# Luolin0826/band

Hardware: AMD Instinct MI355X
Metric: multi-DNN inferences/sec + p99 job latency, 4-model int8 mix @1/2/4/8 GPU (higher is better)
Workload: dtype int8

## Files before the change

band_amd/_abi.py:

```python
import ctypes
import os

_HERE = os.path.dirname(os.path.abspath(__file__))
LIB_PATH = os.path.join(_HERE, "libband_hip%s.so" % (
    "_" + os.environ["BAND_HIP_LIB_VARIANT"] if os.environ.get("BAND_HIP_LIB_VARIANT") else ""))

c_int, c_int32, c_void_p, c_size_t = ctypes.c_int, ctypes.c_int32, ctypes.c_void_p, ctypes.c_size_t


class ConvParams(ctypes.Structure):
    _fields_ = [(n, c_int) for n in (
        "batch", "in_h", "in_w", "in_c", "out_h", "out_w", "out_c", "k_h", "k_w",
        "stride_h", "stride_w", "dil_h", "dil_w", "pad_h", "pad_w", "k_pad", "n_pad", "in_xor")] + [
        (n, c_int32) for n in ("in_zp", "w_zp", "out_zp", "act_min", "act_max")] + [
        (n, c_void_p) for n in ("input", "output", "weights", "bias_eff", "mult", "shift", "residual")] + [
        (n, c_int32) for n in ("add_y_off", "add_r_off", "add_o_off", "add_left_shift", "add_y_mult",
                               "add_y_shift", "add_r_mult", "add_r_shift", "add_o_mult", "add_o_shift",
                               "add_act_min", "add_act_max")] + [("out_table", c_void_p), ("requant_fast", c_int32),
                                                                  ("kernel_hint", c_int32),
                                                                  ("out_img_stride", ctypes.c_int64)]


class ConvGroup(ctypes.Structure):
    _fields_ = [("n", c_int), ("blocks", c_int), ("is1x1", c_int), ("table", c_void_p)]
# ... 36 lines not shown
        "has_expand", "tile_h", "tile_w")] + [
        ("exp_w", c_void_p), ("exp_k_pad", c_int), ("exp_bias_eff", c_void_p), ("exp_mult", c_void_p),
        ("exp_shift", c_void_p)] + [(n, c_int32) for n in ("x_zp", "e_zp", "e_act_min", "e_act_max")] + [
        ("dw_w", c_void_p), ("dw_bias", c_void_p), ("dw_mult", c_void_p), ("dw_shift", c_void_p)] + [
        (n, c_int32) for n in ("d_zp", "d_act_min", "d_act_max")] + [
        ("proj_w", c_void_p), ("proj_k_pad", c_int), ("proj_bias_eff", c_void_p), ("proj_mult", c_void_p),
        ("proj_shift", c_void_p)] + [(n, c_int32) for n in ("p_zp", "p_act_min", "p_act_max")] + [
        ("has_residual", c_int)] + [(n, c_int32) for n in (
            "add_p_off", "add_x_off", "add_o_off", "add_left_shift", "add_p_mult", "add_p_shift", "add_x_mult",
            "add_x_shift", "add_o_mult", "add_o_shift", "add_act_min", "add_act_max")] + [
        ("input", c_void_p), ("output", c_void_p), ("debug_stamps", c_void_p), ("requant_fast", c_int32)]


class MeanParams(ctypes.Structure):
    _fields_ = [(n, ctypes.c_long) for n in ("outer", "reduce", "inner")] + [("type", c_int)] + [
        (n, c_int32) for n in ("multiplier", "shift", "bias")] + [("input", c_void_p), ("output", c_void_p)]


class DetectionParams(ctypes.Structure):
    _fields_ = [(n, c_int) for n in ("batch", "num_boxes", "num_classes", "num_classes_with_background",
                                     "max_detections")] + [
        (n, ctypes.c_float) for n in ("score_threshold", "iou_threshold", "scale_y", "scale_x", "scale_h",
                                      "scale_w")] + [
        ("box_type", c_int), ("score_type", c_int), ("box_scale", ctypes.c_float), ("score_scale", ctypes.c_float),
        ("box_zp", c_int32), ("score_zp", c_int32)] + [
        (n, c_void_p) for n in ("box_encodings", "class_scores", "anchors", "out_boxes", "out_classes",
                                "out_scores", "out_num", "scratch")]


class ChainParams(ctypes.Structure):
    _fields_ = [("dw", DwConvParams), ("pw1", ConvParams), ("pw2", ConvParams), ("has_pw2", c_int),
                ("px_blocks", c_int), ("waves", c_int), ("persist", c_int), ("tile", c_int),
                ("tile_blob", c_void_p), ("debug_stamps", c_void_p), ("deep", c_int), ("c_split", c_int),
                ("stage", c_int)]


CONCAT_MAX_INPUTS = 16


class ConcatParams(ctypes.Structure):
    _fields_ = [("n_inputs", c_int), ("outer", ctypes.c_long),
                ("row", ctypes.c_long * CONCAT_MAX_INPUTS), ("input", c_void_p * CONCAT_MAX_INPUTS),
                ("table", c_void_p * CONCAT_MAX_INPUTS), ("output", c_void_p)]


class PadParams(ctypes.Structure):
    _fields_ = [("elem_bytes", c_int), ("in_shape", c_int * 4), ("pad_before", c_int * 4),
                ("pad_after", c_int * 4), ("value", ctypes.c_uint32), ("input", c_void_p), ("output", c_void_p),
                ("mode", c_int32)]


class ResizeNearestParams(ctypes.Structure):
    _fields_ = [(n, c_int) for n in ("batch", "in_h", "in_w", "out_h", "out_w", "row_bytes")] + [
        (n, c_void_p) for n in ("y_index", "x_index", "input", "output")]


class ResizeBilinearParams(ctypes.Structure):
    _fields_ = [(n, c_int) for n in ("batch", "in_h", "in_w", "channels", "out_h", "out_w")] + [
        (n, c_void_p) for n in ("y_tab", "x_tab", "input", "output")]


ARG_I8, ARG_U8, ARG_F32 = 0, 1, 2


class ArgMinMaxParams(ctypes.Structure):
    _fields_ = [(n, ctypes.c_long) for n in ("outer", "axis_len", "inner")] + [
        (n, c_int) for n in ("in_type", "is_min", "out_bytes")] + [("input", c_void_p), ("output", c_void_p)]
# ... 120 lines not shown
    "bh_argminmax_kernel": (ctypes.c_char_p, [ctypes.POINTER(ArgMinMaxParams)]),
    "bh_resize_bilinear_argminmax_i8": (c_int, [ctypes.POINTER(ResizeArgMinMaxParams), c_void_p]),
    "bh_resize_bilinear_argminmax_i8_ok": (c_int, [ctypes.POINTER(ResizeArgMinMaxParams)]),
    "bh_reindex": (c_int, [ctypes.POINTER(ReindexParams), c_void_p]),
    "bh_reindex_as": (c_int, [ctypes.POINTER(ReindexParams), c_int, c_void_p]),
    "bh_reindex_kernel": (ctypes.c_char_p, [ctypes.POINTER(ReindexParams)]),
    "bh_reindex_canonical": (c_int, [ctypes.POINTER(ReindexParams), ctypes.POINTER(ReindexParams)]),
    "bh_softmax_i8": (c_int, [ctypes.POINTER(SoftmaxParams), c_void_p]),
    "bh_zero_insert": (c_int, [ctypes.POINTER(ZeroInsertParams), c_void_p]),
    "bh_conv2d_f32": (c_int, [ctypes.POINTER(ConvF32Params), c_void_p]),
    "bh_conv2d_f32_split": (c_int, [ctypes.POINTER(ConvF32Params)]),
    "bh_fc_f32": (c_int, [ctypes.POINTER(FcF32Params), c_void_p]),
    "bh_eltwise_f32": (c_int, [ctypes.POINTER(EltwiseF32Params), c_void_p]),
    "bh_pool_f32": (c_int, [ctypes.POINTER(PoolF32Params), c_void_p]),
    "bh_unary_f32": (c_int, [c_int, c_void_p, c_void_p, ctypes.c_long, ctypes.c_float, ctypes.c_float, c_void_p]),
    "bh_softmax_f32": (c_int, [c_void_p, c_void_p, ctypes.c_long, c_int, ctypes.c_float, c_void_p]),
    "bh_dwconv2d_i8": (c_int, [ctypes.POINTER(DwConvParams), c_void_p]),
    "bh_fc_i8": (c_int, [ctypes.POINTER(FcParams), c_void_p]),
    "bh_eltwise_i8": (c_int, [ctypes.POINTER(EltwiseParams), c_void_p]),
    "bh_pool_i8": (c_int, [ctypes.POINTER(PoolParams), c_void_p]),
    "bh_irb_i8": (c_int, [ctypes.POINTER(IrbParams), c_void_p]),
    "bh_irb_lds_bytes": (c_size_t, [ctypes.POINTER(IrbParams)]),
    "bh_chain_i8": (c_int, [ctypes.POINTER(ChainParams), c_void_p]),
    "bh_mean": (c_int, [ctypes.POINTER(MeanParams), c_void_p]),
    "bh_detection_scratch_bytes": (c_size_t, [c_int, c_int]),
    "bh_detection_postprocess": (c_int, [ctypes.POINTER(DetectionParams), c_void_p]),
    "bh_chain_lds_bytes": (c_size_t, [ctypes.POINTER(ChainParams)]),
    "bh_chain_tile_lds_bytes": (c_size_t, [ctypes.POINTER(ChainParams)]),
    "bh_chain_tile_launch": (c_int, [ctypes.POINTER(ChainParams), c_void_p]),
    "bh_chain_tile_blob_bytes": (c_size_t, [ctypes.POINTER(ChainParams)]),
    "bh_chain_tile_pack": (c_int, [ctypes.POINTER(ChainParams), c_void_p, c_void_p]),
    "bh_chain_stage_lds_bytes": (c_size_t, [ctypes.POINTER(ChainParams)]),
    "bh_chain_stage_launch": (c_int, [ctypes.POINTER(ChainParams), c_void_p]),
    "bh_last_error": (ctypes.c_char_p, []),
}

BACKEND_SYMBOLS = {}

_lib = None
_configured = set()


class BandHipError(RuntimeError):
    pass


def load():
    global _lib
    if _lib is None:
        if not os.path.exists(LIB_PATH):
            raise BandHipError(
                "libband_hip.so not built (%s); run __graft_entry__.build() / make -C band_amd/csrc" % LIB_PATH)
        _lib = ctypes.CDLL(LIB_PATH)
    for name, (res, args) in list(KERNEL_SYMBOLS.items()) + list(BACKEND_SYMBOLS.items()):
        if name in _configured:
            continue
        fn = getattr(_lib, name)
        fn.restype = res
        fn.argtypes = args
        _configured.add(name)
    return _lib


def check(rc, what=""):
    if rc != 0:
        msg = load().bh_last_error()
# ... 3 lines not shown
```

band_amd/csrc/backend/hip/chain_form.h:

```cpp
#pragma once

#include "band_hip_kernels.h"

namespace band {
namespace hip {

struct ChainForm {
  int launches;
  int px_blocks, waves, persist, tile, deep, c_split, stage;
};
constexpr bool operator==(const ChainForm& a, const ChainForm& b) {
  return a.launches == b.launches && a.px_blocks == b.px_blocks && a.waves == b.waves && a.persist == b.persist &&
         a.tile == b.tile && a.deep == b.deep && a.c_split == b.c_split && a.stage == b.stage;
}
constexpr ChainForm kUnfused{};
constexpr ChainForm kPlainChain{3, 4, 4, 0, 0, 0, 0, 0};

constexpr ChainForm kChainForms[] = {
    {3, 1, 4, 0, 0, 0, 0, 1}, {3, 1, 8, 0, 0, 0, 0, 1}, {3, 2, 4, 0, 0, 0, 0, 1}, {3, 2, 8, 0, 0, 0, 0, 1},
    {3, 1, 8, 0, 0, 0, 2, 1}, {3, 2, 8, 0, 0, 0, 2, 1}, {3, 1, 8, 0, 0, 0, 4, 1}, {3, 1, 8, 0, 0, 0, 8, 1},
    {3, 1, 8, 0, 0, 0, 0, 2}, {3, 2, 8, 0, 0, 0, 0, 2}, {3, 1, 4, 0, 0, 0, 0, 2}, {3, 1, 8, 0, 0, 0, 2, 2},
    {3, 2, 8, 0, 0, 0, 2, 2}, {3, 1, 8, 0, 0, 0, 3, 2}, {3, 1, 8, 0, 0, 0, 4, 2}, {3, 1, 8, 0, 0, 0, 8, 2},
    {3, 4, 4, 0, 0, 0, 0, 0}, {3, 2, 4, 0, 0, 0, 0, 0}, {3, 1, 4, 0, 0, 0, 0, 0}, {3, 1, 8, 0, 0, 0, 0, 0},
    {3, 1, 16, 0, 0, 0, 0, 0},
    {3, 4, 4, 1, 0, 0, 0, 0}, {3, 4, 4, 0, 1, 0, 0, 0}, {3, 4, 4, 0, 3, 0, 0, 0}, {3, 4, 4, 0, 4, 0, 0, 0},
    {3, 2, 4, 0, 0, 1, 0, 0}, {3, 1, 4, 0, 0, 1, 0, 0}, {3, 1, 8, 0, 0, 1, 0, 0},
    {3, 1, 4, 0, 0, 0, 2, 0}, {3, 1, 8, 0, 0, 0, 2, 0}, {3, 2, 4, 0, 0, 0, 2, 0}, {3, 1, 16, 0, 0, 0, 2, 0},
    {3, 1, 4, 0, 0, 0, 3, 0}, {3, 1, 8, 0, 0, 0, 3, 0}, {3, 1, 4, 0, 0, 0, 4, 0}};

constexpr bool HasLaunches(const ChainForm& f, int launches) {
  return launches == 3 || (launches == 2 && !f.stage && f.c_split <= 1);
}
constexpr bool FilteredOut(const ChainForm& f, bool no_tile, bool no_deep, bool no_split, bool no_stage) {
  return f.stage ? no_stage : (f.tile && no_tile) || (f.deep && no_deep) || (f.c_split && no_split);
}

constexpr int Encode(const ChainForm& f) {
  if (f.launches == 0) return 0;
  if (f.stage) return 100000 + 1000 * (f.stage - 1) + 100 * f.c_split + 10 * f.px_blocks + (f.waves == 8 ? 1 : 0);
  return f.px_blocks + (f.launches == 2 ? 10 : 0) + (f.waves == 16 ? 100 : 0) + (f.waves == 8 ? 300 : 0) +
         (f.persist ? 200 : 0) + (f.tile == 1 ? 400 : 0) + (f.tile == 3 ? 600 : 0) + (f.tile == 4 ? 700 : 0) +
         (f.deep ? 1000 : 0) + (f.c_split > 1 ? 2000 * (f.c_split - 1) : 0);
}
inline bool Decode(int code, ChainForm* out) {
  *out = kUnfused;
  if (code == 0) return true;
  for (ChainForm f : kChainForms)
    for (f.launches = 3; f.launches >= 2; --f.launches)
      if (HasLaunches(f, f.launches) && Encode(f) == code) {
        *out = f;
        return true;
      }
  return false;
}

inline void Apply(const ChainForm& f, bh_chain_params* q) {
  q->px_blocks = f.px_blocks;
  q->waves = f.waves;
  q->persist = f.persist;
  q->tile = f.tile;
  q->deep = f.deep;
  q->c_split = f.c_split;
  q->stage = f.stage;
}
inline bool Fits(ChainForm f, bh_chain_params q) {
  Apply(f, &q);
  return bh_chain_lds_bytes(&q) > 0;
}

enum class ForcedChain { kNone, kPlain, kTile, kDeep, kStage };
inline ChainForm ForcedForm(ForcedChain kind, const bh_chain_params& q) {
  ChainForm plain = kPlainChain, want = kPlainChain;
  plain.launches = want.launches = q.has_pw2 ? 3 : 2;
  if (kind == ForcedChain::kTile) want.tile = 1;
  if (kind == ForcedChain::kDeep) want.px_blocks = want.deep = 1;
  if (kind == ForcedChain::kStage && q.has_pw2) {
    want = ChainForm{3, 1, 8, 0, 0, 0, 2, 1};
    ChainForm loader = want;
    loader.stage = 2;
    if (Fits(want, q) && Fits(loader, q)) want = loader;
  }
  return Fits(want, q) ? want : plain;
}

}
}
```

band_amd/csrc/backend/hip/fusion.cc:

```cpp
#include "backend/hip/chain_form.h"
#include "backend/hip/env.h"
#include "backend/hip/executor_internal.h"
#include <mutex>
#include <optional>
#include <unordered_map>

namespace band {
namespace hip {

using namespace ex;

namespace {
bool LaunchIo(const Launch& l, std::vector<const void*>* rd, std::vector<const void*>* wr) {
  switch (l.kind) {
    case Launch::kConv:
      *rd = {l.conv.input, l.conv.residual};
      *wr = {l.conv.output};
      return true;
    case Launch::kDwConv:
      *rd = {l.dw.input};
      *wr = {l.dw.output};
      return true;
    case Launch::kChain:
      *rd = {l.chain.dw.input, l.chain.pw1.residual};
// ... 444 lines not shown
      out.push_back(L[i]);
      continue;
    }
    std::shared_ptr<DeviceBlob> blob3, blob2;
    auto instantiate = [&](const ChainForm& f, bh_chain_params* q) {
      if (f.launches == 3 ? !ok3 : !ok2) return false;
      *q = f.launches == 3 ? c3 : c2;
      Apply(f, q);
      if (bh_chain_lds_bytes(q) == 0) return false;
      return !(f.tile || f.stage) || PackChainTile(q, f.launches == 3 ? &blob3 : &blob2);
    };
    char key[256];
    std::snprintf(key, sizeof(key), "ch%d:%d:%d:%dx%dx%d:s%dd%d:%d:%d:%d:%d:f%d%d%d%d", kChainTuneVersion, ordinal_,
                  tune_batch_ > 0 ? tune_batch_ : D.dw.batch, D.dw.in_h, D.dw.in_w, D.dw.in_c, D.dw.stride_h, D.dw.dil_h,
                  P1.conv.out_c, P1.conv.residual ? 1 : 0, ok3 ? c3.pw2.out_c : 0, ok3 && c3.pw1.output ? 1 : 0,
                  no_tile_chain_, no_deep_chain_, no_split_chain_, no_stage_chain_);
    const bool forced = forced_chain_ != ForcedChain::kNone;
    const std::optional<int> cached = autotune_ && !forced ? TuneLookup(key) : std::nullopt;
    ChainForm form = kUnfused;
    if (forced) {
      form = ForcedForm(forced_chain_, ok3 ? c3 : c2);
    } else if (cached) {
      Decode(*cached, &form);
    } else {
      std::vector<const Launch*> base = {&D, &P1};
      if (ok3) base.push_back(P2);
      double u = -1.0, u_p2 = 0.0;
      if (autotune_) {
        u = TimeLaunches(base, 10);
        if (ok3) u_p2 = TimeLaunches({P2}, 10);
      }
      const bool measured = u > 0 && u_p2 >= 0;
      Fastest best(u);
      for (ChainForm f : kChainForms) {
        if (!measured || FilteredOut(f, no_tile_chain_, no_deep_chain_, no_split_chain_, no_stage_chain_)) continue;
        for (f.launches = 3; f.launches >= 2; --f.launches) {
          Launch F;
          F.kind = Launch::kChain;
          if (!HasLaunches(f, f.launches) || !instantiate(f, &F.chain)) continue;
          const double us = TimeLaunches({&F}, 10);
          const double total = us + (f.launches == 2 && ok3 ? u_p2 : 0.0);
          if (best.Offer(us > 0 ? total : us)) form = f;
        }
      }
      if (measured) TuneStore(key, Encode(form));
      else form = ForcedForm(ForcedChain::kPlain, ok3 ? c3 : c2);
    }
    Launch F;
    F.kind = Launch::kChain;
    F.op_index = D.op_index;
    if (form.launches == 0 || !instantiate(form, &F.chain)) {
      out.push_back(L[i]);
      continue;
    }
    if (F.chain.tile_blob) sg->consts.push_back(form.launches == 3 ? blob3 : blob2);
    const bool three = form.launches == 3;
    F.out_tensor = three ? P2->out_tensor : P1.out_tensor;
    F.kernel = F.chain.stage ? "chain_stage_kernel" : (F.chain.tile ? "chain_tile_kernel" : "chain_kernel");
    const bh_dwconv_params& dw = F.chain.dw;
    const bh_conv_params& a = F.chain.pw1;
    const double px = static_cast<double>(dw.batch) * dw.out_h * dw.out_w;
    F.alg_bytes = static_cast<double>(dw.batch) * dw.in_h * dw.in_w * dw.in_c + 9.0 * dw.out_c + 28.0 * dw.out_c +
                  (a.residual ? px * a.out_c : 0.0) + (a.output ? px * a.out_c : 0.0) +
                  static_cast<double>(a.out_c) * a.in_c + 12.0 * a.out_c;
    F.alg_ops = D.alg_ops + P1.alg_ops;
    if (three) {
      const bh_conv_params& b = F.chain.pw2;
      F.alg_bytes += px * b.out_c + static_cast<double>(b.out_c) * b.in_c + 12.0 * b.out_c;
      F.alg_ops += P2->alg_ops;
      if (!a.output) sg->fused_tensors.insert(P1.out_tensor);
    }
    out.push_back(F);
    sg->fused_tensors.insert(D.out_tensor);
    i += three ? 2 : 1;
  }
  sg->launches.swap(out);
}

namespace {
void** OutSlot(Launch& l) {
  switch (l.kind) {
    case Launch::kChain: return l.chain.has_pw2 ? &l.chain.pw2.output : &l.chain.pw1.output;
    case Launch::kConv: return &l.conv.output;
    case Launch::kDwConv: return &l.dw.output;
    case Launch::kFc: return &l.fc.output;
    case Launch::kEltwise: return &l.elt.out;
    case Launch::kPool: return &l.pool.output;
    case Launch::kIrb: return &l.irb.output;
    case Launch::kLutU8: return &l.dst;
    default: return nullptr;
  }
// ... 144 lines not shown
```

band_amd/csrc/backend/hip/model_executor.cc:

```cpp
#include "backend/hip/model_executor.h"

#include <sys/prctl.h>
#include <time.h>

#include <chrono>
#include <limits>
#include <mutex>
#include <unordered_map>

#include "backend/hip/affinity.h"
#include "backend/hip/completion.h"
#include "backend/hip/env.h"
#include "backend/hip/executor_internal.h"

namespace band {
namespace hip {

using namespace ex;

namespace ex {
thread_local bool t_variant_ctor = false;
}


// ... 249 lines not shown
  const TflModel& d = model.desc();
  meta_.reserve(d.tensors.size());
  for (const TflTensor& t : d.tensors) {
    auto m = std::make_unique<TensorMeta>();
    m->type = t.type;
    m->dims = t.shape;
    m->name = t.name;
    m->bytes = GetDataTypeBytes(t.type) * t.num_elements();
    m->SetQuant(t.scale, t.zero_point, t.quantized_dimension);
    meta_.push_back(std::move(m));
  }
  consumers_.assign(d.tensors.size(), {});
  producer_.assign(d.tensors.size(), -1);
  for (int i = 0; i < static_cast<int>(d.ops.size()); ++i) {
    for (int t : d.ops[i].inputs)
      if (t >= 0) consumers_[t].push_back(i);
    for (int t : d.ops[i].outputs)
      if (t >= 0) producer_[t] = i;
  }
  const char* f = env::Fusion();
  if (f[0] == '0') allow_fusion_ = false;
  if (std::strcmp(f, "noirb") == 0) allow_irb_ = false;
  if (std::strcmp(f, "noadd") == 0) allow_add_ = false;
  if (std::strcmp(f, "nochain") == 0) allow_chain_ = false;
  if (std::strcmp(f, "nogroup") == 0) allow_group_ = false;
  if (std::strcmp(f, "noargmax") == 0) allow_argmax_ = false;
  if (std::strcmp(f, "forcechain") == 0) forced_chain_ = ForcedChain::kPlain;
  if (std::strcmp(f, "forcetile") == 0) forced_chain_ = ForcedChain::kTile;
  if (std::strcmp(f, "notile") == 0) no_tile_chain_ = true;
  if (std::strcmp(f, "nodeep") == 0) no_deep_chain_ = true;
  if (std::strcmp(f, "nosplit") == 0) no_split_chain_ = true;
  if (std::strcmp(f, "forcedeep") == 0) forced_chain_ = ForcedChain::kDeep;
  if (std::strcmp(f, "forcestage") == 0) forced_chain_ = ForcedChain::kStage;
  if (std::strcmp(f, "nostage") == 0) no_stage_chain_ = true;
  if (!env::Autotune()) autotune_ = false;
  return absl::OkStatus();
}

absl::StatusOr<ModelSpec> HipModelExecutor::InvestigateModelSpec(interface::IModel* model) {
  auto* hm = dynamic_cast<HipModel*>(model);
  if (!hm || !hm->IsInitialized()) return absl::InternalError("Failed to investigate model: not a loaded HIP model");
  const TflModel& d = hm->desc();
  const int num_ops = static_cast<int>(d.ops.size());
  std::vector<DataType> tensor_types;
  std::vector<std::set<int>> op_in, op_out;
  for (const TflOperator& op : d.ops) {
    std::set<int> all, ins, outs;
    for (int t : op.inputs) {
      if (t < 0) continue;
      all.insert(t);
      if (!d.tensors[t].is_const()) ins.insert(t);
    }
    for (int t : op.outputs) {
      if (t < 0) continue;
      all.insert(t);
      if (!d.tensors[t].is_const()) outs.insert(t);
    }
    for (int t : all) tensor_types.push_back(d.tensors[t].type);
    op_in.push_back(ins);
    op_out.push_back(outs);
  }
  std::map<DeviceFlag, std::set<int>> unsupported;
  std::set<DeviceFlag> unavailable;
  const bool gpu = DeviceRegistry::Get().GpuAvailable();
  for (size_t f = 0; f < EnumLength<DeviceFlag>(); ++f) {
    const DeviceFlag flag = static_cast<DeviceFlag>(f);
// ... 617 lines not shown
```

band_amd/csrc/kernels/fused_chain.hip:

```cpp
#include <algorithm>

#include "chain_dw.hpp"
#include "common.hpp"

namespace bh {

__device__ __forceinline__ uint32_t pack4(const int32_t v[4]) {
  const uint32_t lo = __builtin_amdgcn_perm((uint32_t)v[1], (uint32_t)v[0], 0x0c0c0400u);
  const uint32_t hi = __builtin_amdgcn_perm((uint32_t)v[3], (uint32_t)v[2], 0x04000c0cu);
  return lo | hi;
}

__device__ __forceinline__ v4i gemm_tile(const bh_conv_params& c, const unsigned char* xrow, int t, int KS, int r16,
                                         int g) {
  const int8_t* wrow = c.weights + (long)(t * 16 + r16) * c.k_pad + g * 16;
  const int nb = t * 16 + 4 * g;
  const int nl = nb < c.out_c ? nb : 0;
  v4i acc = *(const v4i*)(c.bias_eff + nl);
  int k = 0;
  for (; k + 8 <= KS; k += 8) {
    v4i w[8], x[8];
#pragma unroll
    for (int u = 0; u < 8; ++u) {
      w[u] = *(const v4i*)(wrow + (k + u) * 64);
// ... 771 lines not shown
  return c.k_h == 1 && c.k_w == 1 && c.stride_h == 1 && c.stride_w == 1 && c.pad_h == 0 && c.pad_w == 0 &&
         c.in_c == in_c && c.k_pad == (in_c + 63) / 64 * 64 && c.n_pad >= (c.out_c + 15) / 16 * 16 &&
         c.in_xor == 0 && c.w_zp == 0 && !c.out_table && c.out_c > 0 && c.out_c % 4 == 0 && c.weights &&
         c.bias_eff && c.mult && c.shift;
}

}

extern "C" size_t bh_chain_lds_bytes(const bh_chain_params* pp) {
  if (!pp) return 0;
  const bh_chain_params& p = *pp;
  const bh_dwconv_params& d = p.dw;
  if (!p.tile && !p.stage) {
    if (p.px_blocks != 1 && p.px_blocks != 2 && p.px_blocks != 4) return 0;
    if (p.waves != 0 && p.waves != 4 && !((p.waves == 8 || p.waves == 16) && p.px_blocks == 1)) return 0;
  }
  if (d.k_h != 3 || d.k_w != 3 || d.depth_multiplier != 1 || d.in_c != d.out_c || d.out_c % 16 || !d.taps ||
      d.in_xor != 0 || d.w_zp != 0 || d.out_table || !d.input || !d.weights || !d.mult || !d.shift ||
      d.batch <= 0 || d.out_h <= 0 || d.out_w <= 0 || d.stride_h <= 0 || d.stride_w <= 0)
    return 0;
  if (!bh::conv1x1_ok(p.pw1, d.out_c)) return 0;
  const long P = (long)d.batch * d.out_h * d.out_w;
  if (p.pw1.batch * p.pw1.out_h * p.pw1.out_w != P) return 0;
  if (p.has_pw2) {
    if (!bh::conv1x1_ok(p.pw2, p.pw1.out_c) || p.pw2.residual || !p.pw2.output ||
        p.pw2.k_pad > 64 * bh::kXsMax)
      return 0;
    if ((long)p.pw2.batch * p.pw2.out_h * p.pw2.out_w != P) return 0;
  } else if (!p.pw1.output) {
    return 0;
  }
  const long widest = std::max<long>(std::max(d.out_c, p.pw1.out_c), p.has_pw2 ? p.pw2.out_c : 0);
  if (P * widest >= INT32_MAX || (long)d.batch * d.in_h * d.in_w * d.in_c >= INT32_MAX) return 0;
  if (p.stage) return bh_chain_stage_lds_bytes(pp);
  if (p.c_split < 0 || p.c_split > 4) return 0;
  if (p.c_split > 1 && (p.tile || p.persist || p.deep || p.px_blocks > 2 || !p.has_pw2 ||
                        (p.pw2.out_c + 15) / 16 < p.c_split))
    return 0;
  if (p.tile) return bh_chain_tile_lds_bytes(pp);
  if (p.deep && (p.persist || !((p.px_blocks == 1 && (p.waves == 0 || p.waves == 4 || p.waves == 8)) ||
                                (p.px_blocks == 2 && (p.waves == 0 || p.waves == 4)))))
    return 0;
  if (p.persist) {
    if (p.px_blocks != 4 || (p.waves != 0 && p.waves != 4)) return 0;
    const size_t bytes = bh::persist_lds(p).bytes;
    return bytes <= 160 * 1024 ? bytes : 0;
  }
  bh::ChainLds L = bh::chain_lds(p);
  return L.bytes <= 160 * 1024 ? L.bytes : 0;
}

extern "C" int bh_chain_i8(const bh_chain_params* pp, bh_stream_t stream) {
  const size_t lds = bh_chain_lds_bytes(pp);
  if (lds == 0) {
    bh_set_last_error("bh_chain_i8: invalid or unsupported parameters");
    return BH_EINVAL;
  }
  const bh_chain_params& p = *pp;
  if (p.stage) return bh_chain_stage_launch(pp, stream);
  if (p.tile) return bh_chain_tile_launch(pp, stream);
  const int P = p.dw.batch * p.dw.out_h * p.dw.out_w;
  const bh::ChainLds L = bh::chain_lds(p);
  const bool fast = p.dw.requant_fast && p.pw1.requant_fast && (!p.has_pw2 || p.pw2.requant_fast);
  hipStream_t s = (hipStream_t)stream;
  const bool k2 = !p.has_pw2 || p.pw2.k_pad <= 128;
#define BH_CHAIN_CASE(RB)                                                          \
  if (k2) {                                                                        \
    if (fast) bh::launch_chain<RB, true, 2>(p, P, L, lds, s);                     \
    else bh::launch_chain<RB, false, 2>(p, P, L, lds, s);                         \
  } else {                                                                         \
    if (fast) bh::launch_chain<RB, true, bh::kXsMax>(p, P, L, lds, s);            \
    else bh::launch_chain<RB, false, bh::kXsMax>(p, P, L, lds, s);                \
  }
  if (p.persist) {
    if (k2) {
      if (fast) bh::launch_persist<true, 2>(p, P, lds, s);
      else bh::launch_persist<false, 2>(p, P, lds, s);
    } else {
      if (fast) bh::launch_persist<true, bh::kXsMax>(p, P, lds, s);
      else bh::launch_persist<false, bh::kXsMax>(p, P, lds, s);
    }
    return bh_check_launch("chain_persist_kernel");
  }
  if (p.deep) {
#define BH_DEEP(RB, NW)                                                                      \
  if (k2) {                                                                                  \
    if (fast) bh::launch_chain<RB, true, 2, NW, false, 6>(p, P, L, lds, s);                  \
    else bh::launch_chain<RB, false, 2, NW, false, 6>(p, P, L, lds, s);                      \
  } else {                                                                                   \
    if (fast) bh::launch_chain<RB, true, bh::kXsMax, NW, false, 6>(p, P, L, lds, s);         \
    else bh::launch_chain<RB, false, bh::kXsMax, NW, false, 6>(p, P, L, lds, s);             \
// ... 46 lines not shown
```

include/band_hip_kernels.h:

```cpp
#ifndef BAND_HIP_KERNELS_H_
#define BAND_HIP_KERNELS_H_

#include <stddef.h>
#include <stdint.h>

#ifdef __cplusplus
extern "C" {
#endif

#define BH_EINVAL (-1)

typedef void* bh_stream_t;
typedef void* bh_graph_exec_t;
typedef void* bh_event_t;

int bh_device_count(int* count);
int bh_set_device(int ordinal);
int bh_get_device(int* ordinal);
int bh_device_arch(int ordinal, char* buf, size_t cap);
int bh_device_pci_bus_id(int ordinal, char* buf, int cap);
int bh_stream_create(bh_stream_t* stream);
int bh_stream_destroy(bh_stream_t stream);
int bh_stream_sync(bh_stream_t stream);
int bh_stream_query(bh_stream_t stream);
// ... 162 lines not shown
  const int8_t* dw_w;
  const int32_t* dw_bias; const int32_t* dw_mult; const int32_t* dw_shift;
  int32_t d_zp, d_act_min, d_act_max;
  const int8_t* proj_w; int proj_k_pad;
  const int32_t* proj_bias_eff; const int32_t* proj_mult; const int32_t* proj_shift;
  int32_t p_zp, p_act_min, p_act_max;
  int has_residual;
  int32_t add_p_off, add_x_off, add_o_off, add_left_shift;
  int32_t add_p_mult, add_p_shift, add_x_mult, add_x_shift, add_o_mult, add_o_shift;
  int32_t add_act_min, add_act_max;
  const void* input;
  void* output;
  void* debug_stamps;
  int32_t requant_fast;
} bh_irb_params;

size_t bh_irb_lds_bytes(const bh_irb_params* p);
int bh_irb_i8(const bh_irb_params* p, bh_stream_t s);

typedef struct bh_chain_params {
  bh_dwconv_params dw;
  bh_conv_params pw1;
  bh_conv_params pw2;
  int has_pw2;
  int px_blocks;
  int waves;
  int persist;
  int tile;
  const void* tile_blob;
  void* debug_stamps;
  int deep;
  int c_split;
  int stage;
} bh_chain_params;

size_t bh_chain_lds_bytes(const bh_chain_params* p);
size_t bh_chain_stage_lds_bytes(const bh_chain_params* p);
int bh_chain_stage_launch(const bh_chain_params* p, bh_stream_t s);
size_t bh_chain_tile_lds_bytes(const bh_chain_params* p);
int bh_chain_tile_launch(const bh_chain_params* p, bh_stream_t s);
size_t bh_chain_tile_blob_bytes(const bh_chain_params* p);
int bh_chain_tile_pack(const bh_chain_params* p, void* blob, bh_stream_t s);
int bh_chain_i8(const bh_chain_params* p, bh_stream_t s);

typedef struct bh_mean_params {
  long outer, reduce, inner;
  int type;
  int32_t multiplier, shift, bias;
  const void* input;
  void* output;
} bh_mean_params;
int bh_mean(const bh_mean_params* p, bh_stream_t s);


int bh_pack_conv_weights(const void* w, int w_signed, int out_c, int k,
                         int k_pad, int n_pad, const int32_t* bias,
                         int32_t in_zp, int32_t w_zp, int8_t* packed,
                         int32_t* bias_eff);

int bh_conv_packed_geometry(int out_c, int k, int* k_pad, int* n_pad);
int bh_pack_dw_taps(const int8_t* w, int c, const int32_t* bias, int32_t in_zp, int32_t w_zp, int32_t* taps);
int bh_conv_requant_fast_ok(const int32_t* mult, const int32_t* shift, int n, int k, int64_t max_abs_bias);

int bh_conv2d_i8(const bh_conv_params* p, bh_stream_t s);
const char* bh_conv2d_i8_kernel(const bh_conv_params* p);
int bh_dwconv2d_i8(const bh_dwconv_params* p, bh_stream_t s);
const char* bh_dwconv2d_i8_kernel(const bh_dwconv_params* p);
int bh_fc_i8(const bh_fc_params* p, bh_stream_t s);
int bh_eltwise_i8(const bh_eltwise_params* p, bh_stream_t s);
int bh_pool_i8(const bh_pool_params* p, bh_stream_t s);

// ... 194 lines not shown
```

Measured before the change: 121,300.

## Add dense fused depthwise-pointwise chain kernel as autotuned chain form

Adds a new chain_dense_kernel that runs depthwise conv and one or two pointwise convs per 16-pixel wave, keeping intermediates in a per-wave LDS slab. It uses MFMA for the depthwise taps via lane permutes, and wave-level syncs instead of block barriers. The form is registered in the chain-form list so the autotuner can choose it per layer, and can also be forced via a flag. This aims to cut block-level synchronisation and intermediate traffic in inverted-residual chains, at the cost of more template variants and possible LDS/occupancy pressure.

```diff
diff --git a/band_amd/_abi.py b/band_amd/_abi.py
--- a/band_amd/_abi.py
+++ b/band_amd/_abi.py
@@ -92,7 +92,7 @@
     _fields_ = [("dw", DwConvParams), ("pw1", ConvParams), ("pw2", ConvParams), ("has_pw2", c_int),
                 ("px_blocks", c_int), ("waves", c_int), ("persist", c_int), ("tile", c_int),
                 ("tile_blob", c_void_p), ("debug_stamps", c_void_p), ("deep", c_int), ("c_split", c_int),
-                ("stage", c_int)]
+                ("stage", c_int), ("dense", c_int)]
 
 
 CONCAT_MAX_INPUTS = 16
@@ -279,6 +279,8 @@
     "bh_chain_tile_pack": (c_int, [ctypes.POINTER(ChainParams), c_void_p, c_void_p]),
     "bh_chain_stage_lds_bytes": (c_size_t, [ctypes.POINTER(ChainParams)]),
     "bh_chain_stage_launch": (c_int, [ctypes.POINTER(ChainParams), c_void_p]),
+    "bh_chain_dense_lds_bytes": (c_size_t, [ctypes.POINTER(ChainParams)]),
+    "bh_chain_dense_launch": (c_int, [ctypes.POINTER(ChainParams), c_void_p]),
     "bh_last_error": (ctypes.c_char_p, []),
 }
 
diff --git a/band_amd/csrc/backend/hip/chain_form.h b/band_amd/csrc/backend/hip/chain_form.h
--- a/band_amd/csrc/backend/hip/chain_form.h
+++ b/band_amd/csrc/backend/hip/chain_form.h
@@ -8,10 +8,11 @@
 struct ChainForm {
   int launches;
   int px_blocks, waves, persist, tile, deep, c_split, stage;
+  int dense = 0;
 };
 constexpr bool operator==(const ChainForm& a, const ChainForm& b) {
   return a.launches == b.launches && a.px_blocks == b.px_blocks && a.waves == b.waves && a.persist == b.persist &&
-         a.tile == b.tile && a.deep == b.deep && a.c_split == b.c_split && a.stage == b.stage;
+         a.tile == b.tile && a.deep == b.deep && a.c_split == b.c_split && a.stage == b.stage && a.dense == b.dense;
 }
 constexpr ChainForm kUnfused{};
 constexpr ChainForm kPlainChain{3, 4, 4, 0, 0, 0, 0, 0};
@@ -28,6 +29,14 @@
     {3, 1, 4, 0, 0, 0, 2, 0}, {3, 1, 8, 0, 0, 0, 2, 0}, {3, 2, 4, 0, 0, 0, 2, 0}, {3, 1, 16, 0, 0, 0, 2, 0},
     {3, 1, 4, 0, 0, 0, 3, 0}, {3, 1, 8, 0, 0, 0, 3, 0}, {3, 1, 4, 0, 0, 0, 4, 0}};
 
+constexpr ChainForm kDenseChainForms[] = {{3, 4, 4, 0, 0, 0, 0, 0, 1}};
+
+template <typename Fn>
+inline void ForEachChainForm(Fn&& fn) {
+  for (const ChainForm& f : kChainForms) fn(f);
+  for (const ChainForm& f : kDenseChainForms) fn(f);
+}
+
 constexpr bool HasLaunches(const ChainForm& f, int launches) {
   return launches == 3 || (launches == 2 && !f.stage && f.c_split <= 1);
 }
@@ -40,18 +49,20 @@
   if (f.stage) return 100000 + 1000 * (f.stage - 1) + 100 * f.c_split + 10 * f.px_blocks + (f.waves == 8 ? 1 : 0);
   return f.px_blocks + (f.launches == 2 ? 10 : 0) + (f.waves == 16 ? 100 : 0) + (f.waves == 8 ? 300 : 0) +
          (f.persist ? 200 : 0) + (f.tile == 1 ? 400 : 0) + (f.tile == 3 ? 600 : 0) + (f.tile == 4 ? 700 : 0) +
-         (f.deep ? 1000 : 0) + (f.c_split > 1 ? 2000 * (f.c_split - 1) : 0);
+         (f.deep ? 1000 : 0) + (f.c_split > 1 ? 2000 * (f.c_split - 1) : 0) + (f.dense ? 8000 : 0);
 }
 inline bool Decode(int code, ChainForm* out) {
   *out = kUnfused;
   if (code == 0) return true;
-  for (ChainForm f : kChainForms)
-    for (f.launches = 3; f.launches >= 2; --f.launches)
+  bool found = false;
+  ForEachChainForm([&](ChainForm f) {
+    for (f.launches = 3; f.launches >= 2 && !found; --f.launches)
       if (HasLaunches(f, f.launches) && Encode(f) == code) {
         *out = f;
-        return true;
+        found = true;
       }
-  return false;
+  });
+  return found;
 }
 
 inline void Apply(const ChainForm& f, bh_chain_params* q) {
@@ -62,18 +73,20 @@
   q->deep = f.deep;
   q->c_split = f.c_split;
   q->stage = f.stage;
+  q->dense = f.dense;
 }
 inline bool Fits(ChainForm f, bh_chain_params q) {
   Apply(f, &q);
   return bh_chain_lds_bytes(&q) > 0;
 }
 
-enum class ForcedChain { kNone, kPlain, kTile, kDeep, kStage };
+enum class ForcedChain { kNone, kPlain, kTile, kDeep, kStage, kDense };
 inline ChainForm ForcedForm(ForcedChain kind, const bh_chain_params& q) {
   ChainForm plain = kPlainChain, want = kPlainChain;
   plain.launches = want.launches = q.has_pw2 ? 3 : 2;
   if (kind == ForcedChain::kTile) want.tile = 1;
   if (kind == ForcedChain::kDeep) want.px_blocks = want.deep = 1;
+  if (kind == ForcedChain::kDense) want.dense = 1;
   if (kind == ForcedChain::kStage && q.has_pw2) {
     want = ChainForm{3, 1, 8, 0, 0, 0, 2, 1};
     ChainForm loader = want;
diff --git a/band_amd/csrc/backend/hip/fusion.cc b/band_amd/csrc/backend/hip/fusion.cc
--- a/band_amd/csrc/backend/hip/fusion.cc
+++ b/band_amd/csrc/backend/hip/fusion.cc
@@ -500,8 +500,8 @@
       }
       const bool measured = u > 0 && u_p2 >= 0;
       Fastest best(u);
-      for (ChainForm f : kChainForms) {
-        if (!measured || FilteredOut(f, no_tile_chain_, no_deep_chain_, no_split_chain_, no_stage_chain_)) continue;
+      ForEachChainForm([&](ChainForm f) {
+        if (!measured || FilteredOut(f, no_tile_chain_, no_deep_chain_, no_split_chain_, no_stage_chain_)) return;
         for (f.launches = 3; f.launches >= 2; --f.launches) {
           Launch F;
           F.kind = Launch::kChain;
@@ -510,7 +510,7 @@
           const double total = us + (f.launches == 2 && ok3 ? u_p2 : 0.0);
           if (best.Offer(us > 0 ? total : us)) form = f;
         }
-      }
+      });
       if (measured) TuneStore(key, Encode(form));
       else form = ForcedForm(ForcedChain::kPlain, ok3 ? c3 : c2);
     }
@@ -524,7 +524,9 @@
     if (F.chain.tile_blob) sg->consts.push_back(form.launches == 3 ? blob3 : blob2);
     const bool three = form.launches == 3;
     F.out_tensor = three ? P2->out_tensor : P1.out_tensor;
-    F.kernel = F.chain.stage ? "chain_stage_kernel" : (F.chain.tile ? "chain_tile_kernel" : "chain_kernel");
+    F.kernel = F.chain.dense   ? "chain_dense_kernel"
+               : F.chain.stage ? "chain_stage_kernel"
+                               : (F.chain.tile ? "chain_tile_kernel" : "chain_kernel");
     const bh_dwconv_params& dw = F.chain.dw;
     const bh_conv_params& a = F.chain.pw1;
     const double px = static_cast<double>(dw.batch) * dw.out_h * dw.out_w;
diff --git a/band_amd/csrc/backend/hip/model_executor.cc b/band_amd/csrc/backend/hip/model_executor.cc
--- a/band_amd/csrc/backend/hip/model_executor.cc
+++ b/band_amd/csrc/backend/hip/model_executor.cc
@@ -305,6 +305,7 @@
   if (std::strcmp(f, "nosplit") == 0) no_split_chain_ = true;
   if (std::strcmp(f, "forcedeep") == 0) forced_chain_ = ForcedChain::kDeep;
   if (std::strcmp(f, "forcestage") == 0) forced_chain_ = ForcedChain::kStage;
+  if (std::strcmp(f, "forcedense") == 0) forced_chain_ = ForcedChain::kDense;
   if (std::strcmp(f, "nostage") == 0) no_stage_chain_ = true;
   if (!env::Autotune()) autotune_ = false;
   return absl::OkStatus();
diff --git a/band_amd/csrc/kernels/chain_dense.hip b/band_amd/csrc/kernels/chain_dense.hip
--- /dev/null
+++ b/band_amd/csrc/kernels/chain_dense.hip
@@ -0,0 +1,320 @@
+#include <algorithm>
+#include <climits>
+
+#include "chain_dw.hpp"
+#include "common.hpp"
+
+namespace bh {
+
+struct DenseLds {
+  int S1, S2, slab, off_pl, off_add;
+  size_t bytes;
+};
+
+static DenseLds dense_lds(const bh_chain_params& p) {
+  DenseLds L;
+  L.S1 = p.pw1.k_pad + 32;
+  L.S2 = (p.has_pw2 ? p.pw2.k_pad : (p.pw1.out_c + 15) / 16 * 16) + 32;
+  const int dl_row = std::max(L.S1, p.has_pw2 ? (p.pw2.out_c + 15) / 16 * 16 : 0);
+  L.off_pl = 16 * dl_row;
+  L.slab = L.off_pl + 16 * L.S2;
+  L.off_add = 4 * L.slab;
+  L.bytes = (size_t)L.off_add + (p.pw1.residual ? 512 * sizeof(int) : 0);
+  return L;
+}
+
+__device__ __forceinline__ void dense_copy_rows(const unsigned char* src, int stride, uint8_t* dst, int N, int rows,
+                                                int lane) {
+  const bool v16 = (N & 15) == 0;
+  const int u = v16 ? N >> 4 : N >> 2;
+  const float rcp = 1.0f / (float)u;
+  for (int i = lane; i < rows * u; i += 64) {
+    const int r = (int)(((float)i + 0.5f) * rcp);
+    const int k = i - r * u;
+    if (v16) *(v4i*)(dst + (long)r * N + k * 16) = *(const v4i*)(src + r * stride + k * 16);
+    else *(uint32_t*)(dst + (long)r * N + k * 4) = *(const uint32_t*)(src + r * stride + k * 4);
+  }
+}
+
+struct DenseConv {
+  __amdgpu_buffer_rsrc_t w, be, mu, sh;
+  int wv, cv;
+  int tile_w;
+};
+__device__ __forceinline__ DenseConv dense_conv(const bh_conv_params& c, int r16, int g) {
+  DenseConv d;
+  d.w = __builtin_amdgcn_make_buffer_rsrc((void*)c.weights, (short)0, c.n_pad * c.k_pad, 0x00020000);
+  d.be = __builtin_amdgcn_make_buffer_rsrc((void*)c.bias_eff, (short)0, c.out_c * 4, 0x00020000);
+  d.mu = __builtin_amdgcn_make_buffer_rsrc((void*)c.mult, (short)0, c.out_c * 4, 0x00020000);
+  d.sh = __builtin_amdgcn_make_buffer_rsrc((void*)c.shift, (short)0, c.out_c * 4, 0x00020000);
+  d.wv = r16 * c.k_pad + g * 16;
+  d.cv = r16 * 4;
+  d.tile_w = 16 * c.k_pad;
+  return d;
+}
+template <int KX>
+struct DenseTile {
+  v4i w[KX];
+  int be, mu, sh;
+};
+template <int KX>
+__device__ __forceinline__ void dense_filter_load(const DenseConv& c, int t, int k0, int KS, v4i (&w)[KX]) {
+  typedef unsigned int v4u __attribute__((ext_vector_type(4)));
+#pragma unroll
+  for (int u = 0; u < KX; ++u) {
+    if (k0 + u < KS) {
+      const v4u v = __builtin_amdgcn_raw_buffer_load_b128(c.w, c.wv, t * c.tile_w + (k0 + u) * 64, 0);
+      w[u] = (v4i){(int)v.x, (int)v.y, (int)v.z, (int)v.w};
+    } else {
+      w[u] = (v4i){0, 0, 0, 0};
+    }
+  }
+}
+template <int KX>
+__device__ __forceinline__ void dense_tile_load(const DenseConv& c, int t, int k0, int KS, DenseTile<KX>& d) {
+  dense_filter_load<KX>(c, t, k0, KS, d.w);
+  d.be = (int)__builtin_amdgcn_raw_buffer_load_b32(c.be, c.cv, t * 64, 0);
+  d.mu = (int)__builtin_amdgcn_raw_buffer_load_b32(c.mu, c.cv, t * 64, 0);
+  d.sh = (int)__builtin_amdgcn_raw_buffer_load_b32(c.sh, c.cv, t * 64, 0);
+}
+
+template <bool FAST, bool INTERIOR>
+__device__ __forceinline__ void dense_dw_groups(const bh_dwconv_params& d, const __amdgpu_buffer_rsrc_t rsrc,
+                                                const int (&off)[3], const bool (&ok)[3], bool need, int src4, int r16,
+                                                int g, unsigned char* dl, int S1) {
+  typedef unsigned int v4u __attribute__((ext_vector_type(4)));
+  const int zfill = (int)splat_byte(d.in_zp);
+  const int dsel = r16 >> 2;
+  const int bsh = 8 * (r16 & 3);
+  const int tsel1 = g == 0 ? 0 : 1, tbit1 = g == 0 ? 24 : 8 * (g - 1);
+  const int tbit2 = g < 2 ? 8 * (2 + g) : bsh;
+  const int G = d.out_c >> 4;
+  for (int cg = 0; cg < G; ++cg) {
+    const int c0 = cg * 16;
+    v4u v[3];
+#pragma unroll
+    for (int s = 0; s < 3; ++s) asm volatile("" : "=v"(v[s].x), "=v"(v[s].y), "=v"(v[s].z), "=v"(v[s].w));
+    if (need) {
+#pragma unroll
+      for (int s = 0; s < 3; ++s) v[s] = __builtin_amdgcn_raw_buffer_load_b128(rsrc, off[s] + c0, 0, 0);
+    }
+    const int c = c0 + r16;
+    const v4i tw = *(const v4i*)(d.taps + 4 * c);
+    const int32_t mu = d.mult[c], sh = d.shift[c];
+    v4i xf[3];
+#pragma unroll
+    for (int s = 0; s < 3; ++s) {
+      if (INTERIOR) xf[s] = (v4i){(int)v[s].x, (int)v[s].y, (int)v[s].z, (int)v[s].w};
+      else xf[s] = (v4i){ok[s] ? (int)v[s].x : zfill, ok[s] ? (int)v[s].y : zfill, ok[s] ? (int)v[s].z : zfill,
+                         ok[s] ? (int)v[s].w : zfill};
+#pragma unroll
+      for (int j = 0; j < 4; ++j) xf[s][j] = __builtin_amdgcn_ds_bpermute(src4, xf[s][j]);
+    }
+    const uint32_t t0 = (uint32_t)tw.x, t1 = (uint32_t)tw.y, t2 = (uint32_t)tw.z;
+    uint32_t wb[3];
+    wb[0] = (t0 >> (8 * g)) & 0xffu;
+    wb[1] = ((tsel1 ? t1 : t0) >> tbit1) & 0xffu;
+    wb[2] = ((g < 2 ? t1 : t2) >> tbit2) & 0xffu;
+    v4i acc = (v4i){tw.w, tw.w, tw.w, tw.w};
+#pragma unroll
+    for (int s = 0; s < 3; ++s) {
+      const int w = g < 3 ? (int)(wb[s] << bsh) : 0;
+      const v4i wf = (v4i){dsel == 0 ? w : 0, dsel == 1 ? w : 0, dsel == 2 ? w : 0, dsel == 3 ? w : 0};
+      acc = __builtin_amdgcn_mfma_i32_16x16x64_i8(xf[s], wf, acc, 0, 0, 0);
+    }
+    const ChanQ q = chan_q(mu, sh, d.out_zp);
+    int32_t o[4];
+#pragma unroll
+    for (int r = 0; r < 4; ++r) o[r] = requant_out<FAST>(acc[r], q, d.out_zp, d.act_min, d.act_max);
+    stage4(dl, S1, 4 * g, c, o);
+  }
+}
+
+template <bool FAST>
+__device__ __forceinline__ void dense_dw(const bh_dwconv_params& d, const ChainDivs& dv, int m, bool mval, int lane,
+                                         int r16, int g, unsigned char* dl, int S1) {
+  const int C = d.out_c;
+  const int mm = mval ? m : 0;
+  const int t = dv.out_w.div(mm);
+  const int ox = mm - t * d.out_w;
+  const int n = dv.out_h.div(t);
+  const int oy = t - n * d.out_h;
+  const int iy = oy * d.stride_h, ix = ox * d.stride_w, row0 = n * d.in_h;
+  const int gx = g * d.dil_w;
+  const int dd = (g == 1 || g == 2) && gx % d.stride_w == 0 ? gx / d.stride_w : 0;
+  const bool borrow = dd > 0 && r16 + dd < 16 && ox + dd < d.out_w;
+  const bool need = g < 3 && !borrow;
+  const int src4 = (borrow ? r16 + dd : lane) << 2;
+  int off[3];
+  bool ok[3];
+#pragma unroll
+  for (int s = 0; s < 3; ++s) {
+    const int y = iy + s * d.dil_h - d.pad_h, x = ix + gx - d.pad_w;
+    ok[s] = mval && g < 3 && y >= 0 && y < d.in_h && x >= 0 && x < d.in_w;
+    off[s] = ok[s] ? ((row0 + y) * d.in_w + x) * C : 0;
+  }
+  const __amdgpu_buffer_rsrc_t rsrc =
+      __builtin_amdgcn_make_buffer_rsrc((void*)d.input, (short)0, d.batch * d.in_h * d.in_w * C, 0x00020000);
+  const bool interior = __builtin_amdgcn_ballot_w64(g < 3 && !(ok[0] && ok[1] && ok[2])) == 0;
+  if (interior) dense_dw_groups<FAST, true>(d, rsrc, off, ok, need, src4, r16, g, dl, S1);
+  else dense_dw_groups<FAST, false>(d, rsrc, off, ok, need, src4, r16, g, dl, S1);
+}
+
+__device__ __forceinline__ void dense_wave_sync() {
+  __builtin_amdgcn_fence(__ATOMIC_RELEASE, "wavefront");
+  __builtin_amdgcn_wave_barrier();
+  __builtin_amdgcn_fence(__ATOMIC_ACQUIRE, "wavefront");
+}
+
+template <bool FAST, int KX, int WPE>
+__global__ __launch_bounds__(256, WPE) void chain_dense_kernel(bh_chain_params cp, int P, DenseLds L, ChainDivs dv) {
+  extern __shared__ __attribute__((aligned(16))) unsigned char smem[];
+  const int lane = threadIdx.x & 63;
+  const int pb = threadIdx.x >> 6;
+  const int r16 = lane & 15;
+  const int g = lane >> 4;
+  const int mw = xcd_block(blockIdx.x, gridDim.x) * 64 + pb * 16;
+  unsigned char* dl = smem + pb * L.slab;
+  unsigned char* pl = dl + L.off_pl;
+  const int* add_tab = (const int*)(smem + L.off_add);
+  if (cp.pw1.residual) {
+    const bh_conv_params& a = cp.pw1;
+    int* tab = (int*)(smem + L.off_add);
+    for (int i = threadIdx.x; i < 512; i += 256) {
+      const int q = (i & 255) - 128;
+      tab[i] = i < 256 ? requant_lt1((q + a.add_y_off) * (1 << a.add_left_shift), a.add_y_mult, a.add_y_shift)
+                       : requant_lt1((q + a.add_r_off) * (1 << a.add_left_shift), a.add_r_mult, a.add_r_shift);
+    }
+    __syncthreads();
+  }
+  if (mw >= P) return;
+  const int rows = min(16, P - mw);
+  const int orow = 4 * g;
+
+  dense_dw<FAST>(cp.dw, dv, mw + r16, mw + r16 < P, lane, r16, g, dl, L.S1);
+  dense_wave_sync();
+
+  {
+    const bh_conv_params& a = cp.pw1;
+    const int N1 = a.out_c;
+    const int T1 = (N1 + 15) >> 4;
+    const int KS1 = a.k_pad >> 6;
+    const unsigned char* xrow = dl + r16 * L.S1 + g * 16;
+    const uint8_t* res = (const uint8_t*)a.residual;
+    const DenseConv ac = dense_conv(a, r16, g);
+    for (int t = 0; t < T1; ++t) {
+      DenseTile<2> cur;
+      dense_tile_load<2>(ac, t, 0, KS1, cur);
+      v4i acc = (v4i){cur.be, cur.be, cur.be, cur.be};
+      const int mu = cur.mu, sh = cur.sh;
+      for (int k = 0;;) {
+        acc = __builtin_amdgcn_mfma_i32_16x16x64_i8(*(const v4i*)(xrow + k * 64), cur.w[0], acc, 0, 0, 0);
+        if (k + 1 < KS1)
+          acc = __builtin_amdgcn_mfma_i32_16x16x64_i8(*(const v4i*)(xrow + (k + 1) * 64), cur.w[1], acc, 0, 0, 0);
+        k += 2;
+        if (k >= KS1) break;
+        dense_filter_load<2>(ac, t, k, KS1, cur.w);
+      }
+      const int n = t * 16 + r16;
+      if (n < N1) {
+        const ChanQ q = chan_q(mu, sh, a.out_zp);
+        int32_t v[4];
+#pragma unroll
+        for (int r = 0; r < 4; ++r) v[r] = requant_out<FAST>(acc[r], q, a.out_zp, a.act_min, a.act_max);
+        if (res) {
+          int32_t rq[4];
+#pragma unroll
+          for (int r = 0; r < 4; ++r)
+            rq[r] = (int32_t)(int8_t)res[(uint32_t)(min(mw + orow + r, P - 1) * N1 + n)];
+#pragma unroll
+          for (int r = 0; r < 4; ++r) {
+            const int32_t sy = add_tab[v[r] + 128];
+            const int32_t sr = add_tab[256 + rq[r] + 128];
+            v[r] = clamp_i32(requant_lt1(sy + sr, a.add_o_mult, a.add_o_shift) + a.add_o_off, a.add_act_min,
+                             a.add_act_max);
+          }
+        }
+        stage4(pl, L.S2, orow, n, v);
+      }
+    }
+    dense_wave_sync();
+    if (a.output) dense_copy_rows(pl, L.S2, (uint8_t*)a.output + (long)mw * N1, N1, rows, lane);
+  }
+  if (!cp.has_pw2) return;
+
+  {
+    const bh_conv_params& b = cp.pw2;
+    const int N2 = b.out_c;
+    const int T2 = (N2 + 15) >> 4;
+    const int KS2 = b.k_pad >> 6;
+    v4i x[KX];
+#pragma unroll
+    for (int k = 0; k < KX; ++k) x[k] = k < KS2 ? *(const v4i*)(pl + r16 * L.S2 + g * 16 + k * 64) : (v4i){0, 0, 0, 0};
+    constexpr bool PF = KX <= 2;
+    const DenseConv bc = dense_conv(b, r16, g);
+    DenseTile<KX> cur, nxt;
+    if (PF) dense_tile_load<KX>(bc, 0, 0, KS2, cur);
+    for (int t = 0; t < T2; ++t) {
+      if (!PF) dense_tile_load<KX>(bc, t, 0, KS2, cur);
+      else if (t + 1 < T2) dense_tile_load<KX>(bc, t + 1, 0, KS2, nxt);
+      v4i acc = (v4i){cur.be, cur.be, cur.be, cur.be};
+#pragma unroll
+      for (int k = 0; k < KX; ++k)
+        if (k < KS2) acc = __builtin_amdgcn_mfma_i32_16x16x64_i8(x[k], cur.w[k], acc, 0, 0, 0);
+      const int n = t * 16 + r16;
+      if (n < N2) {
+        const ChanQ q = chan_q(cur.mu, cur.sh, b.out_zp);
+        int32_t v[4];
+#pragma unroll
+        for (int r = 0; r < 4; ++r) v[r] = requant_out<FAST>(acc[r], q, b.out_zp, b.act_min, b.act_max);
+        stage4(dl, N2, orow, n, v);
+      }
+      if (PF && t + 1 < T2) cur = nxt;
+    }
+    dense_wave_sync();
+    dense_copy_rows(dl, N2, (uint8_t*)b.output + (long)mw * N2, N2, rows, lane);
+  }
+}
+
+#ifndef BH_DENSE_WPE
+#define BH_DENSE_WPE 8
+#endif
+
+template <bool FAST, int KX, int WPE>
+static void launch_dense(const bh_chain_params& p, int P, const DenseLds& L, hipStream_t s) {
+  ChainDivs dv;
+  dv.out_w = FastDiv(p.dw.out_w);
+  dv.out_h = FastDiv(p.dw.out_h);
+  BH_LAUNCH((chain_dense_kernel<FAST, KX, WPE>), dim3((P + 63) / 64), dim3(256), L.bytes, s, p, P, L, dv);
+}
+
+}
+
+extern "C" size_t bh_chain_dense_lds_bytes(const bh_chain_params* pp) {
+  const bh_chain_params& p = *pp;
+  if (p.dense != 1 || p.px_blocks != 4 || (p.waves != 0 && p.waves != 4)) return 0;
+  if (p.tile || p.persist || p.deep || p.stage || p.c_split > 1) return 0;
+  if ((long)p.pw1.n_pad * p.pw1.k_pad >= INT32_MAX || (p.has_pw2 && (long)p.pw2.n_pad * p.pw2.k_pad >= INT32_MAX)) return 0;
+  const bh::DenseLds L = bh::dense_lds(p);
+  return L.bytes <= 64 * 1024 ? L.bytes : 0;
+}
+
+extern "C" int bh_chain_dense_launch(const bh_chain_params* pp, bh_stream_t stream) {
+  const bh_chain_params& p = *pp;
+  const int P = p.dw.batch * p.dw.out_h * p.dw.out_w;
+  const bh::DenseLds L = bh::dense_lds(p);
+  const bool fast = p.dw.requant_fast && p.pw1.requant_fast && (!p.has_pw2 || p.pw2.requant_fast);
+  hipStream_t s = (hipStream_t)stream;
+  const int ks2 = p.has_pw2 ? p.pw2.k_pad >> 6 : 1;
+  if (ks2 <= 1) {
+    if (fast) bh::launch_dense<true, 1, BH_DENSE_WPE>(p, P, L, s);
+    else bh::launch_dense<false, 1, BH_DENSE_WPE>(p, P, L, s);
+  } else if (ks2 <= 2) {
+    if (fast) bh::launch_dense<true, 2, BH_DENSE_WPE>(p, P, L, s);
+    else bh::launch_dense<false, 2, BH_DENSE_WPE>(p, P, L, s);
+  } else {
+    if (fast) bh::launch_dense<true, 5, BH_DENSE_WPE>(p, P, L, s);
+    else bh::launch_dense<false, 5, BH_DENSE_WPE>(p, P, L, s);
+  }
+  return bh_check_launch("chain_dense_kernel");
+}
diff --git a/band_amd/csrc/kernels/fused_chain.hip b/band_amd/csrc/kernels/fused_chain.hip
--- a/band_amd/csrc/kernels/fused_chain.hip
+++ b/band_amd/csrc/kernels/fused_chain.hip
@@ -827,6 +827,7 @@
   }
   const long widest = std::max<long>(std::max(d.out_c, p.pw1.out_c), p.has_pw2 ? p.pw2.out_c : 0);
   if (P * widest >= INT32_MAX || (long)d.batch * d.in_h * d.in_w * d.in_c >= INT32_MAX) return 0;
+  if (p.dense) return bh_chain_dense_lds_bytes(pp);
   if (p.stage) return bh_chain_stage_lds_bytes(pp);
   if (p.c_split < 0 || p.c_split > 4) return 0;
   if (p.c_split > 1 && (p.tile || p.persist || p.deep || p.px_blocks > 2 || !p.has_pw2 ||
@@ -852,6 +853,7 @@
     return BH_EINVAL;
   }
   const bh_chain_params& p = *pp;
+  if (p.dense) return bh_chain_dense_launch(pp, stream);
   if (p.stage) return bh_chain_stage_launch(pp, stream);
   if (p.tile) return bh_chain_tile_launch(pp, stream);
   const int P = p.dw.batch * p.dw.out_h * p.dw.out_w;
diff --git a/include/band_hip_kernels.h b/include/band_hip_kernels.h
--- a/include/band_hip_kernels.h
+++ b/include/band_hip_kernels.h
@@ -218,11 +218,14 @@
   int deep;
   int c_split;
   int stage;
+  int dense;
 } bh_chain_params;
 
 size_t bh_chain_lds_bytes(const bh_chain_params* p);
 size_t bh_chain_stage_lds_bytes(const bh_chain_params* p);
 int bh_chain_stage_launch(const bh_chain_params* p, bh_stream_t s);
+size_t bh_chain_dense_lds_bytes(const bh_chain_params* p);
+int bh_chain_dense_launch(const bh_chain_params* p, bh_stream_t s);
 size_t bh_chain_tile_lds_bytes(const bh_chain_params* p);
 int bh_chain_tile_launch(const bh_chain_params* p, bh_stream_t s);
 size_t bh_chain_tile_blob_bytes(const bh_chain_params* p);
```

After: 124,100, median of 6. 2.3% higher.
